# ilur98/DLMC-QUANT

Measured on NVIDIA B200. Metric: fakequant_fwd_bwd_hbm_gbps, higher is better.
Workload: dtype f32

## Files before the change

### dlmc_quant_b200/csrc/fq_kernels.cu

```cuda
#include <mutex>

#include "fq_rows.cuh"

namespace dlmcq {

constexpr int kUnroll = 4;

template <int FORM, typename T, int U = kUnroll, int MINB = 4, bool TILED = false>
__global__ void __launch_bounds__(kThreads, MINB)
fq_fwd_flat(const T* __restrict__ x, T* __restrict__ y, T* __restrict__ codes, int64_t n,
            const float* __restrict__ scale, const float* __restrict__ offset, float g, float lo, float hi,
            int independent) {
  using V = Vec<T>;
  using raw = typename V::raw;
  const int64_t nvec = n / V::N;
  const raw* xv = reinterpret_cast<const raw*>(x);
  const int64_t tile_vecs = static_cast<int64_t>(U) * blockDim.x;
  const int64_t ntiles = nvec / tile_vecs;
  ChanParams p;
  raw r0[U];
  const bool hoist = TILED && independent && blockIdx.x < ntiles;
  if (TILED && independent) {
    p = make_params<FORM>(scale, offset, 0, g, lo, hi);
    if (hoist) {
// ... 44 lines not shown
    }
    for (; i < nvec; i += stride) body(ld_stream(xv + i), i);
  }
  if (blockIdx.x == 0) {
    const int64_t t = nvec * V::N + threadIdx.x;
    if (t < n) {
      float c, v;
      fq_elem<FORM>(to_f32<T>(x[t]), p, lo, hi, c, v);
      if (y) y[t] = from_f32<T>(v);
      if (codes) codes[t] = from_f32<T>(c);
    }
  }
}

template <int FORM, typename T>
__global__ void __launch_bounds__(kThreads)
fq_fwd_flat_unaligned(const T* __restrict__ x, T* __restrict__ y, T* __restrict__ codes, int64_t n,
                      const float* __restrict__ scale, const float* __restrict__ offset, float g, float lo, float hi) {
  const ChanParams p = make_params<FORM>(scale, offset, 0, g, lo, hi);
  const int64_t stride = static_cast<int64_t>(gridDim.x) * blockDim.x;
  for (int64_t i = static_cast<int64_t>(blockIdx.x) * blockDim.x + threadIdx.x; i < n; i += stride) {
    float c, v;
    fq_elem<FORM>(to_f32<T>(x[i]), p, lo, hi, c, v);
    if (y) y[i] = from_f32<T>(v);
    if (codes) codes[i] = from_f32<T>(c);
  }
}

template <int FORM>
__device__ __forceinline__ void finalize_flat(float* partials, int nblocks, float g, float* dscale, float* doffset,
                                              float* smem) {
  double s = 0.0, o = 0.0;
  for (int b = threadIdx.x; b < nblocks; b += blockDim.x) {
    s += static_cast<double>(partials[2 * b]);
    o += static_cast<double>(partials[2 * b + 1]);
  }
  s = warp_sum(s);
  o = warp_sum(o);
  double* sm = reinterpret_cast<double*>(smem);
  const int lane = threadIdx.x & 31, warp = threadIdx.x >> 5, nwarp = blockDim.x >> 5;
  __syncthreads();
  if (lane == 0) { sm[warp] = s; sm[32 + warp] = o; }
  __syncthreads();
  if (threadIdx.x == 0) {
    double ts = 0.0, to = 0.0;
    for (int w = 0; w < nwarp; ++w) { ts += sm[w]; to += sm[32 + w]; }
    float r = static_cast<float>(ts);
    if (FORM == DLMCQ_FORM_AFFINE || FORM == DLMCQ_FORM_A1) r = r * g;
    dscale[0] = r;
    if (doffset) doffset[0] = static_cast<float>(to);
  }
}

template <int FORM, typename T, bool VECTOR, bool WANT_OFF, bool DEFER>
__global__ void __launch_bounds__(kThreads, 4)
fq_bwd_flat(const T* __restrict__ x, const T* __restrict__ dy, T* __restrict__ dx, int64_t n,
            const float* __restrict__ scale, const float* __restrict__ offset, float g, float lo, float hi,
            float* __restrict__ dscale, float* __restrict__ doffset, void* ws, int independent) {
  using V = Vec<T>;
  using raw = typename V::raw;
  __shared__ __align__(16) float smem[128];
  const int64_t nvec = n / V::N;
  const raw* xv = reinterpret_cast<const raw*>(x);
  const raw* gv = reinterpret_cast<const raw*>(dy);
  const int64_t tile_vecs = static_cast<int64_t>(kUnroll) * blockDim.x;
  const int64_t ntiles = nvec / tile_vecs;
  ChanParams p;
  raw rx0[kUnroll], rg0[kUnroll];
  const bool hoist = VECTOR && independent && blockIdx.x < ntiles;
  if (VECTOR && independent) {
    p = make_params<FORM>(scale, offset, 0, g, lo, hi);
    if (hoist) {
      const int64_t b = static_cast<int64_t>(blockIdx.x) * tile_vecs + threadIdx.x;
#pragma unroll
      for (int k = 0; k < kUnroll; ++k) {
        rx0[k] = ld_stream(xv + b + k * blockDim.x);
        rg0[k] = ld_stream(gv + b + k * blockDim.x);
      }
    }
  }
  pdl_wait();
  pdl_trigger();
  if (!(VECTOR && independent)) p = make_params<FORM>(scale, offset, 0, g, lo, hi);
  float acc[2] = {0.f, 0.f};
  const int64_t stride = static_cast<int64_t>(gridDim.x) * blockDim.x;
  int64_t i = static_cast<int64_t>(blockIdx.x) * blockDim.x + threadIdx.x;
  if (VECTOR) {
    raw* ov = reinterpret_cast<raw*>(dx);
    auto body = [&](const raw& rx, const raw& rg, int64_t idx) {
      float fx[V::N], fg[V::N], fo[V::N];
      V::unpack(rx, fx);
      V::unpack(rg, fg);
      fq_vec_bwd<FORM, WANT_OFF, V::N>(fx, fg, p, lo, hi, fo, acc[0], acc[1]);
      st_stream(ov + idx, V::pack(fo));
    };
    int64_t t = blockIdx.x;
    if (hoist) {
      const int64_t b = t * tile_vecs + threadIdx.x;
#pragma unroll
      for (int k = 0; k < kUnroll; ++k) body(rx0[k], rg0[k], b + k * blockDim.x);
      t += gridDim.x;
    }
    for (; t < ntiles; t += gridDim.x) {
      const int64_t b = t * tile_vecs + threadIdx.x;
      raw rx[kUnroll], rg[kUnroll];
#pragma unroll
      for (int k = 0; k < kUnroll; ++k) {
        rx[k] = ld_stream(xv + b + k * blockDim.x);
        rg[k] = ld_stream(gv + b + k * blockDim.x);
      }
#pragma unroll
      for (int k = 0; k < kUnroll; ++k) body(rx[k], rg[k], b + k * blockDim.x);
    }
    for (int64_t j = ntiles * tile_vecs + i; j < nvec; j += stride) body(ld_stream(xv + j), ld_stream(gv + j), j);
    if (blockIdx.x == 0) {
      const int64_t t = nvec * V::N + threadIdx.x;
      if (t < n) dx[t] = from_f32<T>(fq_elem_bwd<FORM, WANT_OFF>(to_f32<T>(x[t]), to_f32<T>(dy[t]), p, lo, hi, acc[0], acc[1]));
    }
  } else {
    for (; i < n; i += stride)
      dx[i] = from_f32<T>(fq_elem_bwd<FORM, WANT_OFF>(to_f32<T>(x[i]), to_f32<T>(dy[i]), p, lo, hi, acc[0], acc[1]));
  }
  block_sum<2>(acc, smem);
  if (DEFER) {
    float* out = static_cast<float*>(ws);
    if (threadIdx.x == 0) {
      if (blockIdx.x == 0) {
        out[0] = __int_as_float(static_cast<int>(gridDim.x));
        out[1] = (FORM == DLMCQ_FORM_AFFINE || FORM == DLMCQ_FORM_A1) ? g : 1.f;
      }
      out[2 + 2 * blockIdx.x] = acc[0];
      out[3 + 2 * blockIdx.x] = acc[1];
    }
    return;
  }
  float* partials = ws_partials(ws);
  if (threadIdx.x == 0) {
    partials[2 * blockIdx.x] = acc[0];
    partials[2 * blockIdx.x + 1] = acc[1];
  }
  if (take_last_ticket(ws_counter(ws), gridDim.x)) {
    finalize_flat<FORM>(partials, gridDim.x, g, dscale, doffset, smem);
    if (threadIdx.x == 0) *ws_counter(ws) = 0u;
  }
}

template <int FORM, typename T>
__global__ void __launch_bounds__(kRowWarps * 32, 3)
fq_fwd_rows(const T* __restrict__ x, T* __restrict__ y, T* __restrict__ codes, RowGeom gm,
            const float* __restrict__ scale, const float* __restrict__ offset, float g, float lo, float hi) {
  const int lane = threadIdx.x & 31;
  const int64_t item = static_cast<int64_t>(blockIdx.x) * kRowWarps + (threadIdx.x >> 5);
  if (item >= gm.rows * gm.segs) return;
  const int64_t row = item / gm.segs, seg = item - row * gm.segs;
  const ChanParams p = make_params<FORM>(scale, offset, row % gm.channels, g, lo, hi);
  const int64_t beg = seg * gm.seg;
  const int64_t len = (gm.inner - beg) < gm.seg ? (gm.inner - beg) : gm.seg;
  const int64_t base = row * gm.inner + beg;
  fwd_row_segment<FORM, T, 8>(x + base, y ? y + base : nullptr, codes ? codes + base : nullptr, len, p, lo, hi, lane);
}

template <int FORM, typename T>
__global__ void __launch_bounds__(kRowWarps * 32)
fq_bwd_rows(const T* __restrict__ x, const T* __restrict__ dy, T* __restrict__ dx, RowGeom gm,
            const float* __restrict__ scale, const float* __restrict__ offset, float g, float lo, float hi,
            float* __restrict__ dscale, float* __restrict__ doffset, float* __restrict__ part, int direct) {
  const int lane = threadIdx.x & 31;
  const int64_t item = static_cast<int64_t>(blockIdx.x) * kRowWarps + (threadIdx.x >> 5);
  if (item >= gm.rows * gm.segs) return;
  const int64_t row = item / gm.segs, seg = item - row * gm.segs;
  const int64_t ch = row % gm.channels;
  const ChanParams p = make_params<FORM>(scale, offset, ch, g, lo, hi);
  const int64_t beg = seg * gm.seg;
  const int64_t len = (gm.inner - beg) < gm.seg ? (gm.inner - beg) : gm.seg;
  const int64_t base = row * gm.inner + beg;
  float as = 0.f, ao = 0.f;
  bwd_row_segment<FORM, T>(x + base, dy + base, dx + base, len, p, lo, hi, lane, as, ao);
  if (lane == 0) {
    if (direct) {
      dscale[ch] = (FORM == DLMCQ_FORM_AFFINE || FORM == DLMCQ_FORM_A1) ? as * g : as;
      if (doffset) doffset[ch] = ao;
    } else {
      part[2 * item] = as;
      part[2 * item + 1] = ao;
    }
  }
}

template <int FORM, typename T, bool BWD, int VEC>
__global__ void __launch_bounds__(kRowWarps * 32, 4)
fq_cmaj_kernel(const T* __restrict__ x, const T* __restrict__ dy, T* __restrict__ out, T* __restrict__ codes,
               CmajGeom gm, const float* __restrict__ scale, const float* __restrict__ offset, float g, float lo,
               float hi, float* __restrict__ dscale, float* __restrict__ part, int direct) {
  using V = Vec<T>;
  using raw = typename V::raw;
// ... 385 lines not shown
      const int64_t tiles = (n / Vec<T>::N + kThreads * kUnroll - 1) / (kThreads * kUnroll);
      auto kern = fq_fwd_flat<FORM, T, kUnroll, 4, true>;
      const int bps = 1024;
      const size_t bytes = static_cast<size_t>(n) * sizeof(T);
      FlatAccess acc;
      acc.read(x, bytes);
      acc.read(qp->scale, sizeof(float));
      acc.read(qp->offset, sizeof(float));
      acc.write(y, bytes);
      acc.write(codes, bytes);
      const int independent = capture_check(st, acc);
      cudaError_t e = launch_pdl(kern, dim3(stream_grid(tiles, bps)), dim3(kThreads), 0, st,
                                 static_cast<const T*>(x), static_cast<T*>(y), static_cast<T*>(codes), n, qp->scale,
                                 qp->offset, qp->g, lo, hi, independent);
      if (e != cudaSuccess) return set_cuda_error(e);
      capture_record(st, acc, independent);
    } else {
      const int64_t tiles = (n + kThreads - 1) / kThreads;
      fq_fwd_flat_unaligned<FORM, T><<<stream_grid(tiles, 8), kThreads, 0, st>>>(
          static_cast<const T*>(x), static_cast<T*>(y), static_cast<T*>(codes), n, qp->scale, qp->offset, qp->g, lo, hi);
    }
  } else if (tiled_ok<T>(l, x, y, codes)) {
    const TileGeom tg = make_tile_geom<T>(l);
    const int64_t tiles = (tg.nvec + kTileVecs - 1) / kTileVecs;
    if (tiles > 0x7fffffffLL) return DLMCQ_EUNSUPPORTED;
    fq_tiled_chan_kernel<FORM, T, false><<<static_cast<unsigned>(tiles), kThreads, 0, st>>>(
        static_cast<const T*>(x), nullptr, static_cast<T*>(y), static_cast<T*>(codes), tg, qp->scale, qp->offset,
        qp->g, lo, hi, nullptr);
  } else if (slab_ok<T>(l->outer, l->channels, l->inner, x, y, codes, nullptr)) {
    const SlabGeom sg = make_slab<T>(l->outer, l->channels, l->inner);
    fq_slab_kernel<FORM, T><<<static_cast<unsigned>(sg.groups) * sg.chunks, kThreads, 0, st>>>(
        static_cast<const T*>(x), static_cast<T*>(y), static_cast<T*>(codes), sg, qp->scale, qp->offset, qp->g, lo, hi);
  } else if (cmaj_ok(l->outer, l->channels, l->inner)) {
    const bool vec = cmaj_vec_ok<T>(l->inner, x, y, codes, nullptr);
    const CmajGeom cg = make_cmaj(l->outer, l->channels, l->inner, vec ? Vec<T>::N : 1);
    const int64_t blocks = (cg.channels * cg.chunks + kRowWarps - 1) / kRowWarps;
    if (blocks > 0x7fffffffLL) return DLMCQ_EUNSUPPORTED;
    auto kern = vec ? fq_cmaj_kernel<FORM, T, false, Vec<T>::N> : fq_cmaj_kernel<FORM, T, false, 1>;
    kern<<<static_cast<unsigned>(blocks), kRowWarps * 32, 0, st>>>(
        static_cast<const T*>(x), nullptr, static_cast<T*>(y), static_cast<T*>(codes), cg, qp->scale, qp->offset,
        qp->g, lo, hi, nullptr, nullptr, 0);
  } else {
    const RowGeom gm = make_geom(l);
    const int64_t items = gm.rows * gm.segs;
    const int64_t blocks = (items + kRowWarps - 1) / kRowWarps;
    if (blocks > 0x7fffffffLL) return DLMCQ_EUNSUPPORTED;
    fq_fwd_rows<FORM, T><<<static_cast<unsigned>(blocks), kRowWarps * 32, 0, st>>>(
        static_cast<const T*>(x), static_cast<T*>(y), static_cast<T*>(codes), gm, qp->scale, qp->offset, qp->g, lo, hi);
  }
  DLMCQ_LAUNCH_CHECK();
  return DLMCQ_OK;
}

template <int FORM, typename T>
static int launch_bwd(const void* x, const void* dy, void* dx, float* dscale, float* doffset, const dlmcq_layout* l,
                      const dlmcq_qparams* qp, void* ws, size_t ws_bytes, cudaStream_t st, bool defer = false) {
  const int64_t n = l->outer * l->channels * l->inner;
  const float lo = static_cast<float>(qp->lo), hi = static_cast<float>(qp->hi);
  if (!defer && ws_bytes < dlmcq_workspace_bytes(l)) return DLMCQ_EWORKSPACE;
  if (defer && l->channels != 1) return DLMCQ_EUNSUPPORTED;
  if (l->channels == 1) {
    const bool vec = aligned16(x) && aligned16(dy) && aligned16(dx);
    const int64_t per = vec ? Vec<T>::N : 1;
    int64_t tiles = (n / per + kThreads * kUnroll - 1) / (kThreads * kUnroll);
    int64_t cap = n < (int64_t(1) << 25) ? 888 : (n < (int64_t(1) << 27) ? 2048 : 4096);
    if (cap > kMaxPartialBlocks) cap = kMaxPartialBlocks;
    const int grid = static_cast<int>(tiles < 1 ? 1 : (tiles < cap ? tiles : cap));
    auto k = vec ? (doffset ? fq_bwd_flat<FORM, T, true, true, false> : fq_bwd_flat<FORM, T, true, false, false>)
                 : (doffset ? fq_bwd_flat<FORM, T, false, true, false> : fq_bwd_flat<FORM, T, false, false, false>);
    if (defer) k = vec ? fq_bwd_flat<FORM, T, true, false, true> : fq_bwd_flat<FORM, T, false, false, true>;
    FlatAccess acc;
    if (vec) {
      const size_t bytes = static_cast<size_t>(n) * sizeof(T);
      acc.read(x, bytes);
      acc.read(dy, bytes);
      acc.read(qp->scale, sizeof(float));
      acc.read(qp->offset, sizeof(float));
      if (!defer) acc.read(ws, ws_bytes);
      acc.write(dx, bytes);
      acc.write(dscale, sizeof(float));
      acc.write(doffset, sizeof(float));
      acc.write(ws, defer ? (2 + 2 * static_cast<size_t>(grid)) * sizeof(float) : ws_bytes);
    }
    const int independent = vec ? capture_check(st, acc) : 0;
    cudaError_t e = launch_pdl(k, dim3(grid), dim3(kThreads), 0, st, static_cast<const T*>(x),
                               static_cast<const T*>(dy), static_cast<T*>(dx), n, qp->scale, qp->offset, qp->g, lo, hi,
                               dscale, doffset, ws, independent);
    if (e != cudaSuccess) return set_cuda_error(e);
    if (vec) capture_record(st, acc, independent);
  } else if (doffset == nullptr && n > 0 && tiled_ok<T>(l, x, dy, dx)) {
    const TileGeom tg = make_tile_geom<T>(l);
    const int64_t tiles = (tg.nvec + kTileVecs - 1) / kTileVecs;
    if (tiles > 0x7fffffffLL) return DLMCQ_EUNSUPPORTED;
    fq_tiled_chan_kernel<FORM, T, true><<<static_cast<unsigned>(tiles), kThreads, 0, st>>>(
        static_cast<const T*>(x), static_cast<const T*>(dy), static_cast<T*>(dx), nullptr, tg, qp->scale, qp->offset,
        qp->g, lo, hi, ws_partials(ws));
    DLMCQ_LAUNCH_CHECK();
    const float gmul = (FORM == DLMCQ_FORM_AFFINE || FORM == DLMCQ_FORM_A1) ? qp->g : 1.f;
    tiled_chan_finalize<<<static_cast<unsigned>(l->channels), 128, 0, st>>>(ws_partials(ws), tg, l->outer, gmul, dscale);
  } else if (cmaj_ok(l->outer, l->channels, l->inner) && doffset == nullptr && n > 0) {
    const bool vec = cmaj_vec_ok<T>(l->inner, x, dy, dx, nullptr);
    const CmajGeom cg = make_cmaj(l->outer, l->channels, l->inner, vec ? Vec<T>::N : 1);
    const int64_t blocks = (cg.channels * cg.chunks + kRowWarps - 1) / kRowWarps;
    if (blocks > 0x7fffffffLL) return DLMCQ_EUNSUPPORTED;
    const int direct = cg.chunks == 1 ? 1 : 0;
    auto kern = vec ? fq_cmaj_kernel<FORM, T, true, Vec<T>::N> : fq_cmaj_kernel<FORM, T, true, 1>;
    kern<<<static_cast<unsigned>(blocks), kRowWarps * 32, 0, st>>>(
        static_cast<const T*>(x), static_cast<const T*>(dy), static_cast<T*>(dx), nullptr, cg, qp->scale, qp->offset,
        qp->g, lo, hi, dscale, ws_partials(ws), direct);
    if (!direct) {
      DLMCQ_LAUNCH_CHECK();
      const float gmul = (FORM == DLMCQ_FORM_AFFINE || FORM == DLMCQ_FORM_A1) ? qp->g : 1.f;
      chan_finalize<1><<<static_cast<unsigned>(cg.channels), 128, 0, st>>>(ws_partials(ws), cg.chunks, cg.chunks, 0,
                                                                           gmul, dscale, nullptr);
    }
  } else {
    const RowGeom gm = make_geom(l);
    const int64_t items = gm.rows * gm.segs;
    const int64_t blocks = (items + kRowWarps - 1) / kRowWarps;
    if (blocks > 0x7fffffffLL) return DLMCQ_EUNSUPPORTED;
    const int direct = (l->outer == 1 && gm.segs == 1) ? 1 : 0;
    if (n == 0) return DLMCQ_OK;
    fq_bwd_rows<FORM, T><<<static_cast<unsigned>(blocks), kRowWarps * 32, 0, st>>>(
        static_cast<const T*>(x), static_cast<const T*>(dy), static_cast<T*>(dx), gm, qp->scale, qp->offset, qp->g,
        lo, hi, dscale, doffset, ws_partials(ws), direct);
    if (!direct) {
      DLMCQ_LAUNCH_CHECK();
      const float gmul = (FORM == DLMCQ_FORM_AFFINE || FORM == DLMCQ_FORM_A1) ? qp->g : 1.f;
      chan_finalize<2><<<static_cast<unsigned>(gm.channels), 128, 0, st>>>(
          ws_partials(ws), l->outer * gm.segs, gm.segs, gm.channels * gm.segs, gmul, dscale, doffset);
    }
  }
  DLMCQ_LAUNCH_CHECK();
  return DLMCQ_OK;
}

template <typename T>
static int dispatch_fwd(const void* x, void* y, void* codes, const dlmcq_layout* l, const dlmcq_qparams* qp,
                        cudaStream_t st) {
  switch (qp->form) {
// ... 138 lines not shown
```

### dlmc_quant_b200/csrc/common.cuh

```cuda
#pragma once
#include <cuda_bf16.h>
#include <cuda_runtime.h>
#include <stdint.h>

#include "../../include/dlmcq.h"

namespace dlmcq {

constexpr int kThreads = 256;
constexpr int kNumSmFallback = 148;
constexpr int kMaxPartialBlocks = 8192;
constexpr int kRowWarps = 8;

int num_sms();
int set_cuda_error(cudaError_t e);
#define DLMCQ_LAUNCH_CHECK()                                   \
  do {                                                         \
    cudaError_t e__ = cudaGetLastError();                      \
    if (e__ != cudaSuccess) return ::dlmcq::set_cuda_error(e__); \
  } while (0)

template <typename T>
struct Vec;
template <>
// ... 3 lines not shown
  __device__ static __forceinline__ void unpack(const raw& r, float (&f)[4]) {
    f[0] = r.x; f[1] = r.y; f[2] = r.z; f[3] = r.w;
  }
  __device__ static __forceinline__ raw pack(const float (&f)[4]) { return make_float4(f[0], f[1], f[2], f[3]); }
};
template <>
struct Vec<__nv_bfloat16> {
  static constexpr int N = 8;
  using raw = uint4;
  __device__ static __forceinline__ void unpack(const raw& r, float (&f)[8]) {
    const uint32_t w[4] = {r.x, r.y, r.z, r.w};
#pragma unroll
    for (int i = 0; i < 4; ++i) {
      f[2 * i] = __uint_as_float(w[i] << 16);
      f[2 * i + 1] = __uint_as_float(w[i] & 0xffff0000u);
    }
  }
  __device__ static __forceinline__ raw pack(const float (&f)[8]) {
    uint32_t w[4];
#pragma unroll
    for (int i = 0; i < 4; ++i) {
      __nv_bfloat162 p = __floats2bfloat162_rn(f[2 * i], f[2 * i + 1]);
      w[i] = *reinterpret_cast<uint32_t*>(&p);
    }
    return make_uint4(w[0], w[1], w[2], w[3]);
  }
};

template <typename T>
__device__ __forceinline__ float to_f32(T v);
template <>
__device__ __forceinline__ float to_f32<float>(float v) { return v; }
template <>
__device__ __forceinline__ float to_f32<__nv_bfloat16>(__nv_bfloat16 v) { return __bfloat162float(v); }
template <typename T>
__device__ __forceinline__ T from_f32(float v);
template <>
__device__ __forceinline__ float from_f32<float>(float v) { return v; }
template <>
__device__ __forceinline__ __nv_bfloat16 from_f32<__nv_bfloat16>(float v) { return __float2bfloat16_rn(v); }

template <typename R>
__device__ __forceinline__ R ld_stream(const R* p) {
  uint4 v;
  asm volatile("ld.global.nc.L1::no_allocate.v4.u32 {%0,%1,%2,%3}, [%4];"
               : "=r"(v.x), "=r"(v.y), "=r"(v.z), "=r"(v.w) : "l"(p));
  return *reinterpret_cast<R*>(&v);
}
template <typename R>
__device__ __forceinline__ void st_stream(R* p, const R& r) {
  const uint4 v = *reinterpret_cast<const uint4*>(&r);
  asm volatile("st.global.L1::no_allocate.v4.u32 [%0], {%1,%2,%3,%4};"
               :: "l"(p), "r"(v.x), "r"(v.y), "r"(v.z), "r"(v.w) : "memory");
}

__device__ __forceinline__ float warp_sum(float v) {
#pragma unroll
  for (int o = 16; o > 0; o >>= 1) v += __shfl_xor_sync(0xffffffffu, v, o);
  return v;
}
__device__ __forceinline__ double warp_sum(double v) {
#pragma unroll
  for (int o = 16; o > 0; o >>= 1) v += __shfl_xor_sync(0xffffffffu, v, o);
  return v;
}
__device__ __forceinline__ float warp_min(float v) {
#pragma unroll
  for (int o = 16; o > 0; o >>= 1) v = fminf(v, __shfl_xor_sync(0xffffffffu, v, o));
  return v;
}
__device__ __forceinline__ float warp_max(float v) {
#pragma unroll
  for (int o = 16; o > 0; o >>= 1) v = fmaxf(v, __shfl_xor_sync(0xffffffffu, v, o));
  return v;
}

template <int NQ>
__device__ __forceinline__ void block_sum(float (&v)[NQ], float* smem ) {
  const int lane = threadIdx.x & 31, warp = threadIdx.x >> 5, nwarp = (blockDim.x + 31) >> 5;
#pragma unroll
  for (int q = 0; q < NQ; ++q) v[q] = warp_sum(v[q]);
  __syncthreads();
  if (lane == 0) {
#pragma unroll
    for (int q = 0; q < NQ; ++q) smem[q * 32 + warp] = v[q];
  }
  __syncthreads();
  if (warp == 0) {
#pragma unroll
    for (int q = 0; q < NQ; ++q) {
      float t = lane < nwarp ? smem[q * 32 + lane] : 0.f;
      v[q] = warp_sum(t);
    }
  }
}

__device__ __forceinline__ bool take_last_ticket(unsigned int* counter, unsigned int nblocks) {
  __shared__ bool is_last;
  if (threadIdx.x == 0) {
    __threadfence();
    unsigned int t = atomicAdd(counter, 1u);
    is_last = (t == nblocks - 1);
  }
  __syncthreads();
  if (is_last) __threadfence();
  return is_last;
// ... 154 lines not shown
```

### dlmc_quant_b200/csrc/fq_rows.cuh

```cuda
#pragma once
#include "fq_math.cuh"

namespace dlmcq {

template <int FORM, typename T, int U = 4>
__device__ __forceinline__ void fwd_row_segment(const T* __restrict__ xr, T* __restrict__ yr, T* __restrict__ cr,
                                                int64_t len, const ChanParams& p, float lo, float hi, int lane) {
  using V = Vec<T>;
  using raw = typename V::raw;
  const bool vec_ok = ((reinterpret_cast<uintptr_t>(xr) | reinterpret_cast<uintptr_t>(yr) |
                        reinterpret_cast<uintptr_t>(cr)) & 15u) == 0;
  int64_t done = 0;
  if (vec_ok) {
    const int64_t nvec = len / V::N;
    const raw* xv = reinterpret_cast<const raw*>(xr);
    auto one = [&](const raw& r, int64_t idx) {
      float f[V::N], fy[V::N], fc[V::N];
      V::unpack(r, f);
      fq_vec<FORM, V::N>(f, p, lo, hi, fc, fy);
      if (yr) st_stream(reinterpret_cast<raw*>(yr) + idx, V::pack(fy));
      if (cr) st_stream(reinterpret_cast<raw*>(cr) + idx, V::pack(fc));
    };
    int64_t j = lane;
    for (; j + 32 * (U - 1) < nvec; j += 32 * U) {
      raw r[U];
#pragma unroll
      for (int h = 0; h < U; ++h) r[h] = ld_stream(xv + j + 32 * h);
#pragma unroll
      for (int h = 0; h < U; ++h) one(r[h], j + 32 * h);
    }
    if (j < nvec) {
      raw r[U];
#pragma unroll
      for (int h = 0; h < U; ++h)
        if (j + 32 * h < nvec) r[h] = ld_stream(xv + j + 32 * h);
#pragma unroll
      for (int h = 0; h < U; ++h)
        if (j + 32 * h < nvec) one(r[h], j + 32 * h);
    }
    done = nvec * V::N;
  }
  for (int64_t j = done + lane; j < len; j += 32) {
    float c, v;
    fq_elem<FORM>(to_f32<T>(xr[j]), p, lo, hi, c, v);
    if (yr) yr[j] = from_f32<T>(v);
    if (cr) cr[j] = from_f32<T>(c);
  }
}

template <int FORM, typename T>
__device__ __forceinline__ void bwd_row_segment(const T* __restrict__ xr, const T* __restrict__ gr,
                                                T* __restrict__ dr, int64_t len, const ChanParams& p, float lo,
                                                float hi, int lane, float& as, float& ao) {
  using V = Vec<T>;
  using raw = typename V::raw;
  const bool vec_ok = ((reinterpret_cast<uintptr_t>(xr) | reinterpret_cast<uintptr_t>(gr) |
                        reinterpret_cast<uintptr_t>(dr)) & 15u) == 0;
  int64_t done = 0;
  if (vec_ok) {
    const int64_t nvec = len / V::N;
    const raw* xv = reinterpret_cast<const raw*>(xr);
    const raw* gv = reinterpret_cast<const raw*>(gr);
    constexpr int U = 4;
    auto one = [&](const raw& rx, const raw& rg, int64_t idx) {
      float fx[V::N], fg[V::N], fo[V::N];
      V::unpack(rx, fx);
      V::unpack(rg, fg);
      fq_vec_bwd<FORM, true, V::N>(fx, fg, p, lo, hi, fo, as, ao);
      st_stream(reinterpret_cast<raw*>(dr) + idx, V::pack(fo));
    };
    int64_t j = lane;
    for (; j + 32 * (U - 1) < nvec; j += 32 * U) {
      raw rx[U], rg[U];
#pragma unroll
      for (int h = 0; h < U; ++h) {
        rx[h] = ld_stream(xv + j + 32 * h);
        rg[h] = ld_stream(gv + j + 32 * h);
      }
#pragma unroll
      for (int h = 0; h < U; ++h) one(rx[h], rg[h], j + 32 * h);
    }
    if (j < nvec) {
      raw rx[U], rg[U];
#pragma unroll
      for (int h = 0; h < U; ++h) {
        if (j + 32 * h < nvec) {
          rx[h] = ld_stream(xv + j + 32 * h);
          rg[h] = ld_stream(gv + j + 32 * h);
        }
      }
#pragma unroll
      for (int h = 0; h < U; ++h)
        if (j + 32 * h < nvec) one(rx[h], rg[h], j + 32 * h);
    }
    done = nvec * V::N;
  }
  for (int64_t j = done + lane; j < len; j += 32)
    dr[j] = from_f32<T>(fq_elem_bwd<FORM, true>(to_f32<T>(xr[j]), to_f32<T>(gr[j]), p, lo, hi, as, ao));
  as = warp_sum(as);
  ao = warp_sum(ao);
}

}
```

### dlmc_quant_b200/csrc/grouped_kernels.cu

```cuda
#include "fq_rows.cuh"

namespace dlmcq {

__device__ __forceinline__ int find_item(const int64_t* __restrict__ prefix, int n_items, int64_t unit) {
  int lo = 0, hi = n_items;
  while (hi - lo > 1) {
    const int mid = (lo + hi) >> 1;
    if (__ldg(prefix + mid) <= unit) lo = mid; else hi = mid;
  }
  return lo;
}

template <int FORM>
__device__ __forceinline__ ChanParams item_params(const dlmcq_group_item& it, int64_t ch) {
  return make_params<FORM>(it.scale, it.offset, ch, it.g, static_cast<float>(it.lo), static_cast<float>(it.hi));
}

template <typename T>
__global__ void __launch_bounds__(kRowWarps * 32)
grouped_fwd_kernel(const dlmcq_group_item* __restrict__ items, const int64_t* __restrict__ prefix, int n_items,
                   int64_t total_units) {
  pdl_wait();
  pdl_trigger();
  const int lane = threadIdx.x & 31;
  const int64_t unit = static_cast<int64_t>(blockIdx.x) * kRowWarps + (threadIdx.x >> 5);
  if (unit >= total_units) return;
  const int k = find_item(prefix, n_items, unit);
  const dlmcq_group_item it = items[k];
  const int64_t local = unit - __ldg(prefix + k);
  const int64_t segs = (it.inner + DLMCQ_GROUP_SEG - 1) / DLMCQ_GROUP_SEG;
  const int64_t row = local / segs, seg = local - row * segs;
  const int64_t beg = seg * DLMCQ_GROUP_SEG;
  const int64_t len = (it.inner - beg) < DLMCQ_GROUP_SEG ? (it.inner - beg) : DLMCQ_GROUP_SEG;
  const T* xr = static_cast<const T*>(it.x) + row * it.inner + beg;
  T* yr = static_cast<T*>(it.y) + row * it.inner + beg;
  const float lo = static_cast<float>(it.lo), hi = static_cast<float>(it.hi);
  switch (it.form) {
    case DLMCQ_FORM_A1: fwd_row_segment<DLMCQ_FORM_A1, T>(xr, yr, nullptr, len, item_params<DLMCQ_FORM_A1>(it, row), lo, hi, lane); break;
    case DLMCQ_FORM_AFFINE: fwd_row_segment<DLMCQ_FORM_AFFINE, T>(xr, yr, nullptr, len, item_params<DLMCQ_FORM_AFFINE>(it, row), lo, hi, lane); break;
    case DLMCQ_FORM_ZP: fwd_row_segment<DLMCQ_FORM_ZP, T>(xr, yr, nullptr, len, item_params<DLMCQ_FORM_ZP>(it, row), lo, hi, lane); break;
    default: fwd_row_segment<DLMCQ_FORM_SYM, T>(xr, yr, nullptr, len, item_params<DLMCQ_FORM_SYM>(it, row), lo, hi, lane); break;
  }
}

template <typename T>
__global__ void __launch_bounds__(kRowWarps * 32)
grouped_bwd_kernel(const dlmcq_group_item* __restrict__ items, const int64_t* __restrict__ prefix, int n_items,
                   int64_t total_units, float* __restrict__ partials) {
  pdl_wait();
  pdl_trigger();
  const int lane = threadIdx.x & 31;
  const int64_t unit = static_cast<int64_t>(blockIdx.x) * kRowWarps + (threadIdx.x >> 5);
  if (unit >= total_units) return;
  const int k = find_item(prefix, n_items, unit);
  const dlmcq_group_item it = items[k];
  const int64_t local = unit - __ldg(prefix + k);
  const int64_t segs = (it.inner + DLMCQ_GROUP_SEG - 1) / DLMCQ_GROUP_SEG;
  const int64_t row = local / segs, seg = local - row * segs;
  const int64_t beg = seg * DLMCQ_GROUP_SEG;
  const int64_t len = (it.inner - beg) < DLMCQ_GROUP_SEG ? (it.inner - beg) : DLMCQ_GROUP_SEG;
  const int64_t base = row * it.inner + beg;
  const T* xr = static_cast<const T*>(it.x) + base;
  const T* gr = static_cast<const T*>(it.dy) + base;
  T* dr = static_cast<T*>(it.y) + base;
  const float lo = static_cast<float>(it.lo), hi = static_cast<float>(it.hi);
  float as = 0.f, ao = 0.f;
  switch (it.form) {
    case DLMCQ_FORM_A1: bwd_row_segment<DLMCQ_FORM_A1, T>(xr, gr, dr, len, item_params<DLMCQ_FORM_A1>(it, row), lo, hi, lane, as, ao); break;
    case DLMCQ_FORM_AFFINE: bwd_row_segment<DLMCQ_FORM_AFFINE, T>(xr, gr, dr, len, item_params<DLMCQ_FORM_AFFINE>(it, row), lo, hi, lane, as, ao); break;
    case DLMCQ_FORM_ZP: bwd_row_segment<DLMCQ_FORM_ZP, T>(xr, gr, dr, len, item_params<DLMCQ_FORM_ZP>(it, row), lo, hi, lane, as, ao); break;
    default: bwd_row_segment<DLMCQ_FORM_SYM, T>(xr, gr, dr, len, item_params<DLMCQ_FORM_SYM>(it, row), lo, hi, lane, as, ao); break;
  }
  if (lane == 0) partials[unit] = as;
}

__global__ void __launch_bounds__(kRowWarps * 32)
grouped_finalize_kernel(const dlmcq_group_item* __restrict__ items, const int64_t* __restrict__ prefix,
                        const int64_t* __restrict__ chan_prefix, int n_items, int64_t total_channels,
                        const float* __restrict__ partials) {
  pdl_wait();
  pdl_trigger();
  const int lane = threadIdx.x & 31;
  const int64_t gch = static_cast<int64_t>(blockIdx.x) * kRowWarps + (threadIdx.x >> 5);
  if (gch >= total_channels) return;
  const int k = find_item(chan_prefix, n_items, gch);
  const dlmcq_group_item it = items[k];
  const int64_t ch = gch - __ldg(chan_prefix + k);
  const int64_t segs = (it.inner + DLMCQ_GROUP_SEG - 1) / DLMCQ_GROUP_SEG;
  const float* p = partials + __ldg(prefix + k) + ch * segs;
  double s = 0.0;
  for (int64_t j = lane; j < segs; j += 32) s += static_cast<double>(p[j]);
  s = warp_sum(s);
  if (lane == 0) {
    float r = static_cast<float>(s);
    if (it.form == DLMCQ_FORM_AFFINE || it.form == DLMCQ_FORM_A1) r = r * it.g;
    it.dscale[ch] = r;
  }
}

}

using namespace dlmcq;

extern "C" int dlmcq_fq_forward_grouped(const dlmcq_group_item* items, const int64_t* unit_prefix, int n_items,
                                        int64_t total_units, int dtype, void* stream) {
  if (!items || !unit_prefix || n_items < 1 || total_units < 0) return DLMCQ_EINVAL;
  if (total_units == 0) return DLMCQ_OK;
  const int64_t blocks = (total_units + kRowWarps - 1) / kRowWarps;
  if (blocks > 0x7fffffffLL) return DLMCQ_EUNSUPPORTED;
  cudaStream_t st = static_cast<cudaStream_t>(stream);
  if (dtype != DLMCQ_F32 && dtype != DLMCQ_BF16) return DLMCQ_EINVAL;
  cudaError_t e = launch_pdl(dtype == DLMCQ_F32 ? grouped_fwd_kernel<float> : grouped_fwd_kernel<__nv_bfloat16>,
                             dim3(static_cast<unsigned>(blocks)), dim3(kRowWarps * 32), 0, st, items, unit_prefix,
                             n_items, total_units);
  if (e != cudaSuccess) return set_cuda_error(e);
  return DLMCQ_OK;
}

extern "C" int dlmcq_fq_backward_grouped(const dlmcq_group_item* items, const int64_t* unit_prefix,
                                         const int64_t* chan_prefix, int n_items, int64_t total_units,
                                         int64_t total_channels, int dtype, float* partials, void* stream) {
  if (!items || !unit_prefix || !chan_prefix || !partials || n_items < 1 || total_units < 0) return DLMCQ_EINVAL;
  if (total_units == 0) return DLMCQ_OK;
  const int64_t blocks = (total_units + kRowWarps - 1) / kRowWarps;
  const int64_t fblocks = (total_channels + kRowWarps - 1) / kRowWarps;
  if (blocks > 0x7fffffffLL || fblocks > 0x7fffffffLL) return DLMCQ_EUNSUPPORTED;
  cudaStream_t st = static_cast<cudaStream_t>(stream);
  if (dtype != DLMCQ_F32 && dtype != DLMCQ_BF16) return DLMCQ_EINVAL;
  cudaError_t e = launch_pdl(dtype == DLMCQ_F32 ? grouped_bwd_kernel<float> : grouped_bwd_kernel<__nv_bfloat16>,
                             dim3(static_cast<unsigned>(blocks)), dim3(kRowWarps * 32), 0, st, items, unit_prefix,
                             n_items, total_units, partials);
  if (e != cudaSuccess) return set_cuda_error(e);
  e = launch_pdl(grouped_finalize_kernel, dim3(static_cast<unsigned>(fblocks)), dim3(kRowWarps * 32), 0, st, items,
                 unit_prefix, chan_prefix, n_items, total_channels, partials);
  if (e != cudaSuccess) return set_cuda_error(e);
  return DLMCQ_OK;
}
```

Measured before the change: 6575.

## Make vectorized bwd kernel persistent with double-buffered tile loads and virtual partials

```diff
diff --git a/dlmc_quant_b200/csrc/fq_kernels.cu b/dlmc_quant_b200/csrc/fq_kernels.cu
--- a/dlmc_quant_b200/csrc/fq_kernels.cu
+++ b/dlmc_quant_b200/csrc/fq_kernels.cu
@@ -120,41 +120,35 @@
   }
 }
 
+constexpr int kBwdCtasPerSm = 2;
+
 template <int FORM, typename T, bool VECTOR, bool WANT_OFF, bool DEFER>
-__global__ void __launch_bounds__(kThreads, 4)
+__global__ void __launch_bounds__(kThreads, VECTOR ? kBwdCtasPerSm : 4)
 fq_bwd_flat(const T* __restrict__ x, const T* __restrict__ dy, T* __restrict__ dx, int64_t n,
             const float* __restrict__ scale, const float* __restrict__ offset, float g, float lo, float hi,
-            float* __restrict__ dscale, float* __restrict__ doffset, void* ws, int independent) {
+            float* __restrict__ dscale, float* __restrict__ doffset, void* ws, int nv, int independent) {
   using V = Vec<T>;
   using raw = typename V::raw;
   __shared__ __align__(16) float smem[128];
-  const int64_t nvec = n / V::N;
-  const raw* xv = reinterpret_cast<const raw*>(x);
-  const raw* gv = reinterpret_cast<const raw*>(dy);
-  const int64_t tile_vecs = static_cast<int64_t>(kUnroll) * blockDim.x;
-  const int64_t ntiles = nvec / tile_vecs;
+  float* out = DEFER ? static_cast<float*>(ws) + 2 : ws_partials(ws);
   ChanParams p;
-  raw rx0[kUnroll], rg0[kUnroll];
-  const bool hoist = VECTOR && independent && blockIdx.x < ntiles;
-  if (VECTOR && independent) {
-    p = make_params<FORM>(scale, offset, 0, g, lo, hi);
-    if (hoist) {
-      const int64_t b = static_cast<int64_t>(blockIdx.x) * tile_vecs + threadIdx.x;
+  float acc[2] = {0.f, 0.f};
+  if (VECTOR) {
+    constexpr int tile_vecs = kThreads * kUnroll;
+    const int64_t nvec = n / V::N;
+    const int64_t ntiles = nvec / tile_vecs;
+    const int64_t vt_end = ntiles < nv ? ntiles : nv;
+    const raw* xv = reinterpret_cast<const raw*>(x);
+    const raw* gv = reinterpret_cast<const raw*>(dy);
+    raw* ov = reinterpret_cast<raw*>(dx);
+    auto load = [&](raw (&rx)[kUnroll], raw (&rg)[kUnroll], int64_t t) {
+      const int64_t b = t * tile_vecs + threadIdx.x;
 #pragma unroll
       for (int k = 0; k < kUnroll; ++k) {
-        rx0[k] = ld_stream(xv + b + k * blockDim.x);
-        rg0[k] = ld_stream(gv + b + k * blockDim.x);
+        rx[k] = ld_stream(xv + b + k * kThreads);
+        rg[k] = ld_stream(gv + b + k * kThreads);
       }
-    }
-  }
-  pdl_wait();
-  pdl_trigger();
-  if (!(VECTOR && independent)) p = make_params<FORM>(scale, offset, 0, g, lo, hi);
-  float acc[2] = {0.f, 0.f};
-  const int64_t stride = static_cast<int64_t>(gridDim.x) * blockDim.x;
-  int64_t i = static_cast<int64_t>(blockIdx.x) * blockDim.x + threadIdx.x;
-  if (VECTOR) {
-    raw* ov = reinterpret_cast<raw*>(dx);
+    };
     auto body = [&](const raw& rx, const raw& rg, int64_t idx) {
       float fx[V::N], fg[V::N], fo[V::N];
       V::unpack(rx, fx);
@@ -162,53 +156,74 @@
       fq_vec_bwd<FORM, WANT_OFF, V::N>(fx, fg, p, lo, hi, fo, acc[0], acc[1]);
       st_stream(ov + idx, V::pack(fo));
     };
-    int64_t t = blockIdx.x;
-    if (hoist) {
+    auto finish = [&](int64_t v) {
+      for (int64_t j = ntiles * tile_vecs + v * kThreads + threadIdx.x; j < nvec; j += static_cast<int64_t>(nv) * kThreads)
+        body(ld_stream(xv + j), ld_stream(gv + j), j);
+      if (v == 0) {
+        const int64_t t = nvec * V::N + threadIdx.x;
+        if (t < n) dx[t] = from_f32<T>(fq_elem_bwd<FORM, WANT_OFF>(to_f32<T>(x[t]), to_f32<T>(dy[t]), p, lo, hi, acc[0], acc[1]));
+      }
+      block_sum<2>(acc, smem);
+      if (threadIdx.x == 0) {
+        out[2 * v] = acc[0];
+        out[2 * v + 1] = acc[1];
+      }
+      acc[0] = acc[1] = 0.f;
+    };
+    raw ax[kUnroll], ag[kUnroll], bx[kUnroll], bg[kUnroll];
+    int64_t v = blockIdx.x, t = blockIdx.x;
+    bool more = v < vt_end;
+    if (independent) {
+      p = make_params<FORM>(scale, offset, 0, g, lo, hi);
+      if (more) load(ax, ag, t);
+    }
+    pdl_wait();
+    pdl_trigger();
+    if (!independent) {
+      p = make_params<FORM>(scale, offset, 0, g, lo, hi);
+      if (more) load(ax, ag, t);
+    }
+    auto step = [&](raw (&cx)[kUnroll], raw (&cg)[kUnroll], raw (&nx)[kUnroll], raw (&ng)[kUnroll]) {
+      int64_t v2 = v, t2 = t + nv;
+      if (t2 >= ntiles) t2 = v2 = v + gridDim.x;
+      more = v2 < vt_end;
+      if (more) load(nx, ng, t2);
       const int64_t b = t * tile_vecs + threadIdx.x;
 #pragma unroll
-      for (int k = 0; k < kUnroll; ++k) body(rx0[k], rg0[k], b + k * blockDim.x);
-      t += gridDim.x;
-    }
-    for (; t < ntiles; t += gridDim.x) {
-      const int64_t b = t * tile_vecs + threadIdx.x;
-      raw rx[kUnroll], rg[kUnroll];
-#pragma unroll
-      for (int k = 0; k < kUnroll; ++k) {
-        rx[k] = ld_stream(xv + b + k * blockDim.x);
-        rg[k] = ld_stream(gv + b + k * blockDim.x);
-      }
-#pragma unroll
-      for (int k = 0; k < kUnroll; ++k) body(rx[k], rg[k], b + k * blockDim.x);
-    }
-    for (int64_t j = ntiles * tile_vecs + i; j < nvec; j += stride) body(ld_stream(xv + j), ld_stream(gv + j), j);
-    if (blockIdx.x == 0) {
-      const int64_t t = nvec * V::N + threadIdx.x;
-      if (t < n) dx[t] = from_f32<T>(fq_elem_bwd<FORM, WANT_OFF>(to_f32<T>(x[t]), to_f32<T>(dy[t]), p, lo, hi, acc[0], acc[1]));
-    }
+      for (int k = 0; k < kUnroll; ++k) body(cx[k], cg[k], b + k * kThreads);
+      if (v2 != v) finish(v);
+      v = v2;
+      t = t2;
+    };
+    while (more) {
+      step(ax, ag, bx, bg);
+      if (!more) break;
+      step(bx, bg, ax, ag);
+    }
+    for (; v < nv; v += gridDim.x) finish(v);
   } else {
-    for (; i < n; i += stride)
+    pdl_wait();
+    pdl_trigger();
+    p = make_params<FORM>(scale, offset, 0, g, lo, hi);
+    const int64_t stride = static_cast<int64_t>(gridDim.x) * blockDim.x;
+    for (int64_t i = static_cast<int64_t>(blockIdx.x) * blockDim.x + threadIdx.x; i < n; i += stride)
       dx[i] = from_f32<T>(fq_elem_bwd<FORM, WANT_OFF>(to_f32<T>(x[i]), to_f32<T>(dy[i]), p, lo, hi, acc[0], acc[1]));
-  }
-  block_sum<2>(acc, smem);
+    block_sum<2>(acc, smem);
+    if (threadIdx.x == 0) {
+      out[2 * blockIdx.x] = acc[0];
+      out[2 * blockIdx.x + 1] = acc[1];
+    }
+  }
   if (DEFER) {
-    float* out = static_cast<float*>(ws);
-    if (threadIdx.x == 0) {
-      if (blockIdx.x == 0) {
-        out[0] = __int_as_float(static_cast<int>(gridDim.x));
-        out[1] = (FORM == DLMCQ_FORM_AFFINE || FORM == DLMCQ_FORM_A1) ? g : 1.f;
-      }
-      out[2 + 2 * blockIdx.x] = acc[0];
-      out[3 + 2 * blockIdx.x] = acc[1];
+    if (threadIdx.x == 0 && blockIdx.x == 0) {
+      float* hdr = static_cast<float*>(ws);
+      hdr[0] = __int_as_float(nv);
+      hdr[1] = (FORM == DLMCQ_FORM_AFFINE || FORM == DLMCQ_FORM_A1) ? g : 1.f;
     }
     return;
   }
-  float* partials = ws_partials(ws);
-  if (threadIdx.x == 0) {
-    partials[2 * blockIdx.x] = acc[0];
-    partials[2 * blockIdx.x + 1] = acc[1];
-  }
   if (take_last_ticket(ws_counter(ws), gridDim.x)) {
-    finalize_flat<FORM>(partials, gridDim.x, g, dscale, doffset, smem);
+    finalize_flat<FORM>(out, nv, g, dscale, doffset, smem);
     if (threadIdx.x == 0) *ws_counter(ws) = 0u;
   }
 }
@@ -700,6 +715,22 @@
   return DLMCQ_OK;
 }
 
+template <int FORM, typename T, bool WANT_OFF, bool DEFER>
+static int bwd_resident_ctas() {
+  static int cached[64] = {0};
+  int dev = 0;
+  cudaError_t e = cudaGetDevice(&dev);
+  if (e == cudaSuccess && dev >= 0 && dev < 64 && cached[dev] > 0) return cached[dev];
+  int per_sm = 0;
+  if (e == cudaSuccess)
+    e = cudaOccupancyMaxActiveBlocksPerMultiprocessor(&per_sm, fq_bwd_flat<FORM, T, true, WANT_OFF, DEFER>, kThreads, 0);
+  if (e != cudaSuccess) return set_cuda_error(e), 0;
+  if (per_sm <= 0) return set_cuda_error(cudaErrorInvalidConfiguration), 0;
+  const int ctas = num_sms() * per_sm;
+  if (dev >= 0 && dev < 64) cached[dev] = ctas;
+  return ctas;
+}
+
 template <int FORM, typename T>
 static int launch_bwd(const void* x, const void* dy, void* dx, float* dscale, float* doffset, const dlmcq_layout* l,
                       const dlmcq_qparams* qp, void* ws, size_t ws_bytes, cudaStream_t st, bool defer = false) {
@@ -713,10 +744,18 @@
     int64_t tiles = (n / per + kThreads * kUnroll - 1) / (kThreads * kUnroll);
     int64_t cap = n < (int64_t(1) << 25) ? 888 : (n < (int64_t(1) << 27) ? 2048 : 4096);
     if (cap > kMaxPartialBlocks) cap = kMaxPartialBlocks;
-    const int grid = static_cast<int>(tiles < 1 ? 1 : (tiles < cap ? tiles : cap));
+    const int nv = static_cast<int>(tiles < 1 ? 1 : (tiles < cap ? tiles : cap));
     auto k = vec ? (doffset ? fq_bwd_flat<FORM, T, true, true, false> : fq_bwd_flat<FORM, T, true, false, false>)
                  : (doffset ? fq_bwd_flat<FORM, T, false, true, false> : fq_bwd_flat<FORM, T, false, false, false>);
     if (defer) k = vec ? fq_bwd_flat<FORM, T, true, false, true> : fq_bwd_flat<FORM, T, false, false, true>;
+    int grid = nv;
+    if (vec) {
+      const int resident = defer     ? bwd_resident_ctas<FORM, T, false, true>()
+                           : doffset ? bwd_resident_ctas<FORM, T, true, false>()
+                                     : bwd_resident_ctas<FORM, T, false, false>();
+      if (resident <= 0) return DLMCQ_ECUDA;
+      if (grid > resident) grid = resident;
+    }
     FlatAccess acc;
     if (vec) {
       const size_t bytes = static_cast<size_t>(n) * sizeof(T);
@@ -728,12 +767,12 @@
       acc.write(dx, bytes);
       acc.write(dscale, sizeof(float));
       acc.write(doffset, sizeof(float));
-      acc.write(ws, defer ? (2 + 2 * static_cast<size_t>(grid)) * sizeof(float) : ws_bytes);
+      acc.write(ws, defer ? (2 + 2 * static_cast<size_t>(nv)) * sizeof(float) : ws_bytes);
     }
     const int independent = vec ? capture_check(st, acc) : 0;
     cudaError_t e = launch_pdl(k, dim3(grid), dim3(kThreads), 0, st, static_cast<const T*>(x),
                                static_cast<const T*>(dy), static_cast<T*>(dx), n, qp->scale, qp->offset, qp->g, lo, hi,
-                               dscale, doffset, ws, independent);
+                               dscale, doffset, ws, nv, independent);
     if (e != cudaSuccess) return set_cuda_error(e);
     if (vec) capture_record(st, acc, independent);
   } else if (doffset == nullptr && n > 0 && tiled_ok<T>(l, x, dy, dx)) {
diff --git a/profiles/bwd_sweep.py b/profiles/bwd_sweep.py
--- /dev/null
+++ b/profiles/bwd_sweep.py
@@ -0,0 +1,76 @@
+import argparse
+import ctypes as C
+import json
+import math
+import os
+import sys
+
+ROOT = os.path.dirname(os.path.dirname(os.path.abspath(__file__)))
+if ROOT not in sys.path:
+    sys.path.insert(0, ROOT)
+
+SIZES = [262144, 3211264, 6422528, 12845056, 19267584, 25690112, 51380224, 102760448]
+L2_BYTES = 126 << 20
+
+
+def main():
+    ap = argparse.ArgumentParser()
+    ap.add_argument("--lib", default=None)
+    ap.add_argument("--label", default="this")
+    ap.add_argument("--iters", type=int, default=200)
+    ap.add_argument("--out", default=None)
+    args = ap.parse_args()
+    import torch
+
+    from dlmc_quant_b200 import _lib
+    if args.lib:
+        _lib.LIB_PATH = os.path.abspath(args.lib)
+    h = _lib.lib()
+    assert os.path.samefile(_lib.LIB_PATH, args.lib or _lib.LIB_PATH)
+    dev = torch.device("cuda")
+    gen = torch.Generator(device=dev).manual_seed(2333)
+    st = C.c_void_p(torch.cuda.current_stream().cuda_stream)
+    lo, hi = 0, 15
+    rows = []
+    for n in SIZES:
+        sets = max(1, math.ceil(3 * L2_BYTES / (12 * n)))
+        bufs = []
+        for _ in range(sets):
+            x = torch.relu(torch.randn(n, generator=gen, device=dev)) * 2
+            bufs.append((x, torch.randn(n, generator=gen, device=dev), torch.empty(n, device=dev),
+                         torch.empty(h.dlmcq_fq_partials_floats(), device=dev)))
+        scale = torch.full((1,), float(bufs[0][0].max()) / hi, device=dev)
+        off = torch.zeros(1, device=dev)
+        lay = _lib.Layout(1, 1, n, _lib.F32)
+        qp = _lib.QParams(_lib.FORM_AFFINE, lo, hi, 1 / math.sqrt(n * hi), scale.data_ptr(), off.data_ptr())
+        f = h.dlmcq_fq_backward_partials
+
+        def launch(i):
+            x, dy, dx, parts = bufs[i % sets]
+            _lib.check(f(x.data_ptr(), dy.data_ptr(), dx.data_ptr(), C.byref(lay), C.byref(qp), parts.data_ptr(), st))
+
+        for i in range(20):
+            launch(i)
+        torch.cuda.synchronize()
+        t0, t1 = torch.cuda.Event(enable_timing=True), torch.cuda.Event(enable_timing=True)
+        t0.record()
+        for i in range(args.iters):
+            launch(i)
+        t1.record()
+        torch.cuda.synchronize()
+        us = t0.elapsed_time(t1) * 1e3 / args.iters
+        nv = int(bufs[0][3][:1].view(torch.int32).item())
+        row = {"label": args.label, "n": n, "partials": nv, "sets": sets, "us_per_launch": round(us, 2),
+               "tb_s": round(12 * n / (us * 1e-6) / 1e12, 3), "gpu": torch.cuda.get_device_name()}
+        rows.append(row)
+        print(json.dumps(row), flush=True)
+        del bufs
+        torch.cuda.empty_cache()
+    if args.out:
+        with open(args.out, "a") as fo:
+            for r in rows:
+                fo.write(json.dumps(r) + "\n")
+
+
+if __name__ == "__main__":
+    main()
```

After: 6500 (median of 6 runs). -1.1%, worse.

## Add L2 eviction hints, reverse backward order, and warp-parallel item lookup

Applied to the files above, without the earlier changes.

```diff
diff --git a/dlmc_quant_b200/csrc/common.cuh b/dlmc_quant_b200/csrc/common.cuh
--- a/dlmc_quant_b200/csrc/common.cuh
+++ b/dlmc_quant_b200/csrc/common.cuh
@@ -79,6 +79,30 @@
   const uint4 v = *reinterpret_cast<const uint4*>(&r);
   asm volatile("st.global.L1::no_allocate.v4.u32 [%0], {%1,%2,%3,%4};"
                :: "l"(p), "r"(v.x), "r"(v.y), "r"(v.z), "r"(v.w) : "memory");
+}
+
+__device__ __forceinline__ uint64_t l2_evict_first() {
+  uint64_t p;
+  asm("createpolicy.fractional.L2::evict_first.b64 %0, 1.0;" : "=l"(p));
+  return p;
+}
+__device__ __forceinline__ uint64_t l2_evict_last() {
+  uint64_t p;
+  asm("createpolicy.fractional.L2::evict_last.b64 %0, 1.0;" : "=l"(p));
+  return p;
+}
+template <typename R>
+__device__ __forceinline__ R ld_stream_hint(const R* p, uint64_t pol) {
+  uint4 v;
+  asm volatile("ld.global.nc.L1::no_allocate.L2::cache_hint.v4.u32 {%0,%1,%2,%3}, [%4], %5;"
+               : "=r"(v.x), "=r"(v.y), "=r"(v.z), "=r"(v.w) : "l"(p), "l"(pol));
+  return *reinterpret_cast<R*>(&v);
+}
+template <typename R>
+__device__ __forceinline__ void st_stream_hint(R* p, const R& r, uint64_t pol) {
+  const uint4 v = *reinterpret_cast<const uint4*>(&r);
+  asm volatile("st.global.L1::no_allocate.L2::cache_hint.v4.u32 [%0], {%1,%2,%3,%4}, %5;"
+               :: "l"(p), "r"(v.x), "r"(v.y), "r"(v.z), "r"(v.w), "l"(pol) : "memory");
 }
 
 __device__ __forceinline__ float warp_sum(float v) {
diff --git a/dlmc_quant_b200/csrc/fq_rows.cuh b/dlmc_quant_b200/csrc/fq_rows.cuh
--- a/dlmc_quant_b200/csrc/fq_rows.cuh
+++ b/dlmc_quant_b200/csrc/fq_rows.cuh
@@ -3,9 +3,14 @@
 
 namespace dlmcq {
 
-template <int FORM, typename T, int U = 4>
+struct RowPolicy {
+  uint64_t in, out;
+};
+
+template <int FORM, typename T, int U = 4, bool HINT = false>
 __device__ __forceinline__ void fwd_row_segment(const T* __restrict__ xr, T* __restrict__ yr, T* __restrict__ cr,
-                                                int64_t len, const ChanParams& p, float lo, float hi, int lane) {
+                                                int64_t len, const ChanParams& p, float lo, float hi, int lane,
+                                                RowPolicy pol = {0, 0}) {
   using V = Vec<T>;
   using raw = typename V::raw;
   const bool vec_ok = ((reinterpret_cast<uintptr_t>(xr) | reinterpret_cast<uintptr_t>(yr) |
@@ -18,14 +23,18 @@
       float f[V::N], fy[V::N], fc[V::N];
       V::unpack(r, f);
       fq_vec<FORM, V::N>(f, p, lo, hi, fc, fy);
-      if (yr) st_stream(reinterpret_cast<raw*>(yr) + idx, V::pack(fy));
+      if (yr) {
+        if (HINT) st_stream_hint(reinterpret_cast<raw*>(yr) + idx, V::pack(fy), pol.out);
+        else st_stream(reinterpret_cast<raw*>(yr) + idx, V::pack(fy));
+      }
       if (cr) st_stream(reinterpret_cast<raw*>(cr) + idx, V::pack(fc));
     };
+    auto load = [&](int64_t idx) { return HINT ? ld_stream_hint(xv + idx, pol.in) : ld_stream(xv + idx); };
     int64_t j = lane;
     for (; j + 32 * (U - 1) < nvec; j += 32 * U) {
       raw r[U];
 #pragma unroll
-      for (int h = 0; h < U; ++h) r[h] = ld_stream(xv + j + 32 * h);
+      for (int h = 0; h < U; ++h) r[h] = load(j + 32 * h);
 #pragma unroll
       for (int h = 0; h < U; ++h) one(r[h], j + 32 * h);
     }
@@ -33,7 +42,7 @@
       raw r[U];
 #pragma unroll
       for (int h = 0; h < U; ++h)
-        if (j + 32 * h < nvec) r[h] = ld_stream(xv + j + 32 * h);
+        if (j + 32 * h < nvec) r[h] = load(j + 32 * h);
 #pragma unroll
       for (int h = 0; h < U; ++h)
         if (j + 32 * h < nvec) one(r[h], j + 32 * h);
@@ -48,10 +57,10 @@
   }
 }
 
-template <int FORM, typename T>
+template <int FORM, typename T, bool HINT = false>
 __device__ __forceinline__ void bwd_row_segment(const T* __restrict__ xr, const T* __restrict__ gr,
                                                 T* __restrict__ dr, int64_t len, const ChanParams& p, float lo,
-                                                float hi, int lane, float& as, float& ao) {
+                                                float hi, int lane, float& as, float& ao, RowPolicy pol = {0, 0}) {
   using V = Vec<T>;
   using raw = typename V::raw;
   const bool vec_ok = ((reinterpret_cast<uintptr_t>(xr) | reinterpret_cast<uintptr_t>(gr) |
@@ -67,15 +76,17 @@
       V::unpack(rx, fx);
       V::unpack(rg, fg);
       fq_vec_bwd<FORM, true, V::N>(fx, fg, p, lo, hi, fo, as, ao);
-      st_stream(reinterpret_cast<raw*>(dr) + idx, V::pack(fo));
+      if (HINT) st_stream_hint(reinterpret_cast<raw*>(dr) + idx, V::pack(fo), pol.out);
+      else st_stream(reinterpret_cast<raw*>(dr) + idx, V::pack(fo));
     };
+    auto load = [&](const raw* v, int64_t idx) { return HINT ? ld_stream_hint(v + idx, pol.in) : ld_stream(v + idx); };
     int64_t j = lane;
     for (; j + 32 * (U - 1) < nvec; j += 32 * U) {
       raw rx[U], rg[U];
 #pragma unroll
       for (int h = 0; h < U; ++h) {
-        rx[h] = ld_stream(xv + j + 32 * h);
-        rg[h] = ld_stream(gv + j + 32 * h);
+        rx[h] = load(xv, j + 32 * h);
+        rg[h] = load(gv, j + 32 * h);
       }
 #pragma unroll
       for (int h = 0; h < U; ++h) one(rx[h], rg[h], j + 32 * h);
@@ -85,8 +96,8 @@
 #pragma unroll
       for (int h = 0; h < U; ++h) {
         if (j + 32 * h < nvec) {
-          rx[h] = ld_stream(xv + j + 32 * h);
-          rg[h] = ld_stream(gv + j + 32 * h);
+          rx[h] = load(xv, j + 32 * h);
+          rg[h] = load(gv, j + 32 * h);
         }
       }
 #pragma unroll
diff --git a/dlmc_quant_b200/csrc/grouped_kernels.cu b/dlmc_quant_b200/csrc/grouped_kernels.cu
--- a/dlmc_quant_b200/csrc/grouped_kernels.cu
+++ b/dlmc_quant_b200/csrc/grouped_kernels.cu
@@ -9,6 +9,20 @@
     if (__ldg(prefix + mid) <= unit) lo = mid; else hi = mid;
   }
   return lo;
+}
+
+__device__ __forceinline__ int find_item_warp(const int64_t* __restrict__ prefix, int n_items, int64_t unit, int lane) {
+  if (n_items > 128) return find_item(prefix, n_items, unit);
+  int64_t p[4];
+#pragma unroll
+  for (int c = 0; c < 4; ++c) {
+    const int k = c * 32 + lane;
+    p[c] = k < n_items ? __ldg(prefix + k) : INT64_MAX;
+  }
+  int cnt = 0;
+#pragma unroll
+  for (int c = 0; c < 4; ++c) cnt += __popc(__ballot_sync(0xffffffffu, p[c] <= unit));
+  return cnt - 1;
 }
 
 template <int FORM>
@@ -25,7 +39,7 @@
   const int lane = threadIdx.x & 31;
   const int64_t unit = static_cast<int64_t>(blockIdx.x) * kRowWarps + (threadIdx.x >> 5);
   if (unit >= total_units) return;
-  const int k = find_item(prefix, n_items, unit);
+  const int k = find_item_warp(prefix, n_items, unit, lane);
   const dlmcq_group_item it = items[k];
   const int64_t local = unit - __ldg(prefix + k);
   const int64_t segs = (it.inner + DLMCQ_GROUP_SEG - 1) / DLMCQ_GROUP_SEG;
@@ -35,11 +49,12 @@
   const T* xr = static_cast<const T*>(it.x) + row * it.inner + beg;
   T* yr = static_cast<T*>(it.y) + row * it.inner + beg;
   const float lo = static_cast<float>(it.lo), hi = static_cast<float>(it.hi);
+  const RowPolicy pol = {l2_evict_last(), l2_evict_first()};
   switch (it.form) {
-    case DLMCQ_FORM_A1: fwd_row_segment<DLMCQ_FORM_A1, T>(xr, yr, nullptr, len, item_params<DLMCQ_FORM_A1>(it, row), lo, hi, lane); break;
-    case DLMCQ_FORM_AFFINE: fwd_row_segment<DLMCQ_FORM_AFFINE, T>(xr, yr, nullptr, len, item_params<DLMCQ_FORM_AFFINE>(it, row), lo, hi, lane); break;
-    case DLMCQ_FORM_ZP: fwd_row_segment<DLMCQ_FORM_ZP, T>(xr, yr, nullptr, len, item_params<DLMCQ_FORM_ZP>(it, row), lo, hi, lane); break;
-    default: fwd_row_segment<DLMCQ_FORM_SYM, T>(xr, yr, nullptr, len, item_params<DLMCQ_FORM_SYM>(it, row), lo, hi, lane); break;
+    case DLMCQ_FORM_A1: fwd_row_segment<DLMCQ_FORM_A1, T, 4, true>(xr, yr, nullptr, len, item_params<DLMCQ_FORM_A1>(it, row), lo, hi, lane, pol); break;
+    case DLMCQ_FORM_AFFINE: fwd_row_segment<DLMCQ_FORM_AFFINE, T, 4, true>(xr, yr, nullptr, len, item_params<DLMCQ_FORM_AFFINE>(it, row), lo, hi, lane, pol); break;
+    case DLMCQ_FORM_ZP: fwd_row_segment<DLMCQ_FORM_ZP, T, 4, true>(xr, yr, nullptr, len, item_params<DLMCQ_FORM_ZP>(it, row), lo, hi, lane, pol); break;
+    default: fwd_row_segment<DLMCQ_FORM_SYM, T, 4, true>(xr, yr, nullptr, len, item_params<DLMCQ_FORM_SYM>(it, row), lo, hi, lane, pol); break;
   }
 }
 
@@ -50,9 +65,10 @@
   pdl_wait();
   pdl_trigger();
   const int lane = threadIdx.x & 31;
-  const int64_t unit = static_cast<int64_t>(blockIdx.x) * kRowWarps + (threadIdx.x >> 5);
-  if (unit >= total_units) return;
-  const int k = find_item(prefix, n_items, unit);
+  const int64_t rev = static_cast<int64_t>(blockIdx.x) * kRowWarps + (threadIdx.x >> 5);
+  if (rev >= total_units) return;
+  const int64_t unit = total_units - 1 - rev;
+  const int k = find_item_warp(prefix, n_items, unit, lane);
   const dlmcq_group_item it = items[k];
   const int64_t local = unit - __ldg(prefix + k);
   const int64_t segs = (it.inner + DLMCQ_GROUP_SEG - 1) / DLMCQ_GROUP_SEG;
@@ -65,11 +81,12 @@
   T* dr = static_cast<T*>(it.y) + base;
   const float lo = static_cast<float>(it.lo), hi = static_cast<float>(it.hi);
   float as = 0.f, ao = 0.f;
+  const RowPolicy pol = {l2_evict_first(), l2_evict_first()};
   switch (it.form) {
-    case DLMCQ_FORM_A1: bwd_row_segment<DLMCQ_FORM_A1, T>(xr, gr, dr, len, item_params<DLMCQ_FORM_A1>(it, row), lo, hi, lane, as, ao); break;
-    case DLMCQ_FORM_AFFINE: bwd_row_segment<DLMCQ_FORM_AFFINE, T>(xr, gr, dr, len, item_params<DLMCQ_FORM_AFFINE>(it, row), lo, hi, lane, as, ao); break;
-    case DLMCQ_FORM_ZP: bwd_row_segment<DLMCQ_FORM_ZP, T>(xr, gr, dr, len, item_params<DLMCQ_FORM_ZP>(it, row), lo, hi, lane, as, ao); break;
-    default: bwd_row_segment<DLMCQ_FORM_SYM, T>(xr, gr, dr, len, item_params<DLMCQ_FORM_SYM>(it, row), lo, hi, lane, as, ao); break;
+    case DLMCQ_FORM_A1: bwd_row_segment<DLMCQ_FORM_A1, T, true>(xr, gr, dr, len, item_params<DLMCQ_FORM_A1>(it, row), lo, hi, lane, as, ao, pol); break;
+    case DLMCQ_FORM_AFFINE: bwd_row_segment<DLMCQ_FORM_AFFINE, T, true>(xr, gr, dr, len, item_params<DLMCQ_FORM_AFFINE>(it, row), lo, hi, lane, as, ao, pol); break;
+    case DLMCQ_FORM_ZP: bwd_row_segment<DLMCQ_FORM_ZP, T, true>(xr, gr, dr, len, item_params<DLMCQ_FORM_ZP>(it, row), lo, hi, lane, as, ao, pol); break;
+    default: bwd_row_segment<DLMCQ_FORM_SYM, T, true>(xr, gr, dr, len, item_params<DLMCQ_FORM_SYM>(it, row), lo, hi, lane, as, ao, pol); break;
   }
   if (lane == 0) partials[unit] = as;
 }
@@ -83,7 +100,7 @@
   const int lane = threadIdx.x & 31;
   const int64_t gch = static_cast<int64_t>(blockIdx.x) * kRowWarps + (threadIdx.x >> 5);
   if (gch >= total_channels) return;
-  const int k = find_item(chan_prefix, n_items, gch);
+  const int k = find_item_warp(chan_prefix, n_items, gch, lane);
   const dlmcq_group_item it = items[k];
   const int64_t ch = gch - __ldg(chan_prefix + k);
   const int64_t segs = (it.inner + DLMCQ_GROUP_SEG - 1) / DLMCQ_GROUP_SEG;
diff --git a/profiles/weight_path.py b/profiles/weight_path.py
--- /dev/null
+++ b/profiles/weight_path.py
@@ -0,0 +1,57 @@
+import argparse
+import json
+import os
+import sys
+
+ROOT = os.path.dirname(os.path.dirname(os.path.abspath(__file__)))
+if ROOT not in sys.path:
+    sys.path.insert(0, ROOT)
+
+
+def main():
+    ap = argparse.ArgumentParser()
+    ap.add_argument("--iters", type=int, default=200)
+    ap.add_argument("--out", default=None)
+    args = ap.parse_args()
+    import torch
+
+    import bench
+    wl = bench.Workload(1, torch.device("cuda"), 2333)
+    wl.capture()
+    g_f = torch.cuda.CUDAGraph()
+    with torch.cuda.graph(g_f):
+        wl.grp_f.forward(wl.wf)
+    flush = torch.empty(256 << 20, dtype=torch.uint8, device="cuda")
+
+    def timed(graph, evict):
+        for _ in range(10):
+            graph.replay()
+        torch.cuda.synchronize()
+        total = 0.0
+        for _ in range(args.iters):
+            if evict:
+                flush.add_(1)
+            a, b = torch.cuda.Event(enable_timing=True), torch.cuda.Event(enable_timing=True)
+            a.record()
+            graph.replay()
+            b.record()
+            b.synchronize()
+            total += a.elapsed_time(b) * 1e3
+        return total / args.iters
+
+    n = wl.wt_elems
+    res = {"gpu": torch.cuda.get_device_name(), "weight_elems": n, "iters": args.iters}
+    for evict in (True, False):
+        key = "cold_l2" if evict else "back_to_back"
+        us_all, us_f = timed(wl.g_wt, evict), timed(g_f, evict)
+        gbs_all, gbs_f = 20 * n / us_all / 1e3, 8 * n / us_f / 1e3
+        res[key] = {"fwd_bwd_fin_us": round(us_all, 2), "fwd_us": round(us_f, 2), "fwd_bwd_fin_GBps": round(gbs_all, 1),
+                    "fwd_GBps": round(gbs_f, 1), "share_of_fwd_rate": round(gbs_all / gbs_f, 3)}
+    print(json.dumps(res), flush=True)
+    if args.out:
+        with open(args.out, "w") as f:
+            json.dump(res, f, indent=1)
+
+
+if __name__ == "__main__":
+    main()
```

Measured after the change: 6577 before, 6624 after (median of 6 runs). About the same (+0.7%).
